# noegroup/bgflow

Measured on AMD Instinct MI355X. Metric: flow samples/s (fwd+log|detJ|) at batch 2^20, higher is better.
Workload: dtype f32 (split-f16 conditioner GEMMs: hi+lo f16 operand pairs, f32 accumulate)

## Files before the change

bgflow_amd/build.py:

```python
import glob
import os
import subprocess
import sys
from concurrent.futures import ThreadPoolExecutor

HERE = os.path.dirname(os.path.abspath(__file__))
CSRC = os.path.join(HERE, "csrc")
OBJ = os.path.join(CSRC, "build")
LIB = os.path.join(HERE, "libbgflow_amd.so")

HIPCC_FLAGS = [
    "--offload-arch=gfx950", "-O3", "-std=c++17", "-fPIC", "-fvisibility=hidden",
    "-ffp-contract=off", "-fhip-fp32-correctly-rounded-divide-sqrt", "-fno-fast-math",
    "-Wno-comment",
]
TU_FLAGS = {"bgk_fused2.hip": ["-fno-slp-vectorize"], "bgk_fused2_train.hip": ["-fno-slp-vectorize"],
            "bgk_fused2_bf16.hip": ["-fno-slp-vectorize"], "bgk_fused2_afftrain.hip": ["-fno-slp-vectorize"],
            "bgk_tail.hip": ["-fno-slp-vectorize"]}


INCLUDES_SOURCE = {"bgk_fused2_train.hip": ["bgk_fused2.hip"], "bgk_fused2_bf16.hip": ["bgk_fused2.hip"], "bgk_fused2_afftrain.hip": ["bgk_fused2.hip"]}


HEADER = os.path.join(HERE, "..", "include", "bgflow_amd.h")


def abi_symbols(header=HEADER):
    import re
    text = re.sub(r"/\*.*?\*/", "", open(header).read(), flags=re.S)
    return sorted(set(re.findall(r"^[A-Za-z_][\w \t\*]*?\b(bgk_\w+)\s*\(", text, flags=re.M)))


def _export_map():
    path = os.path.join(OBJ, "export.map")
    with open(path, "w") as f:
        f.write("{\n  global:\n" + "".join(f"    {n};\n" for n in abi_symbols()) + "  local:\n    *;\n};\n")
    return path


def sources():
    return sorted(glob.glob(os.path.join(CSRC, "*.hip")))


def _headers():
    return glob.glob(os.path.join(CSRC, "*.h")) + glob.glob(os.path.join(HERE, "..", "include", "*.h"))


def _obj(src, tag):
    return os.path.join(OBJ, os.path.basename(src) + tag + ".o")


def _stale():
    if not os.path.exists(LIB):
        return True
# ... 40 lines not shown
```

bgflow_amd/csrc/bgk_capi.hip:

```cpp
#include <stdarg.h>

#include "bgk_common.h"
#include "bgk_fused2.h"

extern int bgk_affine_variant;

static thread_local char g_err[512] = "";

void bgk_set_error(const char* fmt, ...) {
    va_list ap;
    va_start(ap, fmt);
    vsnprintf(g_err, sizeof(g_err), fmt, ap);
    va_end(ap);
}

extern "C" int bgk_abi_version(void) { return 1; }
extern "C" const char* bgk_last_error(void) { return g_err; }

extern "C" int bgk_set_option(int32_t option, int32_t value) {
    if (option == 1 && (value == 1 || value == 2)) {
        const int prev = bgk_h2_variant;
        bgk_h2_variant = value;
        return prev;
    }
    if (option == 2 && (value == 1 || value == 2)) {
        const int prev = bgk_affine_variant;
        bgk_affine_variant = value;
        return prev;
    }
    if (option == 3 && (value == 1 || value == 2)) {
        const int prev = bgk_rc_vjp_variant;
        bgk_rc_vjp_variant = value;
        return prev;
    }
    bgk_set_error("bgk_set_option: unknown option %d / value %d", option, value);
    return BGK_EINVAL;
}

namespace {
__global__ void detmath_probe_kernel(const float* x, int64_t n, int which, float* out) {
    int64_t i = (int64_t)blockIdx.x * blockDim.x + threadIdx.x;
    if (i >= n) return;
    float v = x[i], r;
    switch (which) {
        case 0: r = bgk_expf(v); break;
        case 1: r = bgk_logf(v); break;
        case 2: r = bgk_softplusf(v, 0.69384102162f); break;
        case 3: r = bgk_siluf(v); break;
        case 4: r = bgk_tanhf(v); break;
        default: r = v;
    }
    out[i] = r;
}
}

extern "C" int bgk_detmath_probe(const float* x, int64_t n, int32_t which, float* out, void* stream) {
    if (n <= 0) return 0;
    int grid = (int)((n + 255) / 256);
    hipLaunchKernelGGL(detmath_probe_kernel, dim3(grid), dim3(256), 0, (hipStream_t)stream, x, n, which, out);
    return bgk_launch_status("bgk_detmath_probe");
}
```

bgflow_amd/csrc/bgk_fused2.h:

```cpp
#ifndef BGK_FUSED2_H
#define BGK_FUSED2_H
#include <stdint.h>

#define BGK_MAX_COND 3
struct BgkCondSegs { const float* ptr[BGK_MAX_COND]; int64_t ld[BGK_MAX_COND]; int32_t w[BGK_MAX_COND]; int32_t n; };

int bgk_launch_rqs_dense_h2v2(const char* what, const float* cond, int64_t ldc, int32_t d_c, int32_t periodic,
                              const void* A0p, const void* A1p, const void* A2p, float c0, float c1, float c2, const float* cs_dev,
                              int32_t act, const float* y, int64_t ldy, int64_t B, int32_t d, uint64_t circ_mask, int32_t inverse,
                              double left, double right, double bottom, double top,
                              double min_bin_width, double min_bin_height, double min_derivative, int32_t identity_init,
                              float* out, int64_t ldo, float* dlogp, int32_t accumulate, int32_t* bin_idx, int32_t* oob_count,
                              void* stream, const BgkCondSegs* segs = nullptr, int32_t row_order = 1);

int bgk_launch_rqs_dense_h2v2_train(const char* what, float* z0, float* z1, float* params, int64_t ldp, const int32_t* src_col,
                                    const float* cond, int64_t ldc, int32_t d_c, int32_t periodic,
                                    const void* A0p, const void* A1p, const void* A2p, float c0, float c1, float c2, const float* cs_dev,
                                    int32_t act, const float* y, int64_t ldy, int64_t B, int32_t d, uint64_t circ_mask, int32_t inverse,
                                    double left, double right, double bottom, double top,
                                    double min_bin_width, double min_bin_height, double min_derivative, int32_t identity_init,
                                    float* out, int64_t ldo, float* dlogp, int32_t accumulate, int32_t* bin_idx, int32_t* oob_count,
                                    void* stream, const BgkCondSegs* segs = nullptr, int32_t row_order = 1);

int bgk_launch_rqs_bwd_recompute(const char* what, const float* z1, const void* A2p, float c2, const float* cs_dev, int32_t act,
                                 const float* y, int64_t ldy, int64_t B, int32_t d, uint64_t circ_mask, int32_t inverse,
                                 double left, double right, double bottom, double top,
                                 double min_bin_width, double min_bin_height, double min_derivative, int32_t identity_init,
                                 const float* g_out, int64_t ldgo, const float* g_dlogp, float* g_y, int64_t ldgy,
                                 float* g_params, int64_t ldgp, float* g_absmax, void* stream);

int bgk_launch_rqs_dense_h2v2_bf16(const char* what, const float* cond, int64_t ldc, int32_t d_c, int32_t periodic,
                                   const void* A0p, const void* A1p, const void* A2p, float c0, float c1, float c2, const float* cs_dev,
                                   int32_t act, const float* y, int64_t ldy, int64_t B, int32_t d, uint64_t circ_mask, int32_t inverse,
                                   double left, double right, double bottom, double top,
                                   double min_bin_width, double min_bin_height, double min_derivative, int32_t identity_init,
                                   float* out, int64_t ldo, float* dlogp, int32_t accumulate, int32_t* bin_idx, int32_t* oob_count,
                                   void* stream, const BgkCondSegs* segs = nullptr, int32_t row_order = 1);

int bgk_launch_affine_dense_v2(const float* cond, int64_t ldc, int32_t d_c, int32_t periodic,
                               const void* sA0, const void* sA1, const void* sA1b, const void* sA2, float sc0, float sc1, float sc1b, float sc2, int32_t s_act,
                               const void* tA0, const void* tA1, const void* tA1b, const void* tA2, float tc0, float tc1, float tc1b, float tc2, int32_t t_act,
                               const float* log_alpha, int32_t preserve_volume, int32_t is_circular, int32_t inverse,
                               const float* y, int64_t ldy, int64_t B, int32_t d,
                               float* out, int64_t ldo, float* dlogp, int32_t accumulate, void* stream, const BgkCondSegs* segs = nullptr);

struct BgkAffTrainSave { const float* s_cs; float* s_z0; float* s_z1; const float* t_cs; float* t_z0; float* t_z1; float* mu; float* s_raw; int64_t ldms;
                         int64_t ldz; };
int bgk_launch_affine_dense_v2_train(const BgkAffTrainSave* save, const float* cond, int64_t ldc, int32_t d_c, int32_t periodic,
                               const void* sA0, const void* sA1, const void* sA1b, const void* sA2, float sc0, float sc1, float sc1b, float sc2, int32_t s_act,
                               const void* tA0, const void* tA1, const void* tA1b, const void* tA2, float tc0, float tc1, float tc1b, float tc2, int32_t t_act,
                               const float* log_alpha, int32_t preserve_volume, int32_t is_circular, int32_t inverse,
                               const float* y, int64_t ldy, int64_t B, int32_t d,
                               float* out, int64_t ldo, float* dlogp, int32_t accumulate, void* stream, const BgkCondSegs* segs = nullptr);

extern int bgk_h2_variant;
extern int bgk_rc_vjp_variant;

#endif
```

bgflow_amd/csrc/bgk_fused2.hip:

```cpp
#include "bgk_common.h"
#include "bgk_fused2.h"

#ifndef BGK_V2_SAVE
#define BGK_V2_SAVE 0
#endif
#if BGK_V2_SAVE
#include "bgk_mfma_h2.h"
#include "bgk_rqs_vjp.h"
#define coupling_rqs_dense_h2v2_kernel coupling_rqs_dense_h2v2_train_kernel
#endif
#ifndef BGK_V2_BF16
#define BGK_V2_BF16 0
#endif
#if BGK_V2_BF16
#define coupling_rqs_dense_h2v2_kernel coupling_rqs_dense_h2v2_bf16_kernel
typedef short s16x8 __attribute__((ext_vector_type(8)));
#endif
#ifndef BGK_V2_AFFTRAIN
#define BGK_V2_AFFTRAIN 0
#endif
#if BGK_V2_AFFTRAIN
#define coupling_affine_dense_v2_kernel coupling_affine_dense_v2_train_kernel
#endif
constexpr int NPROD = BGK_V2_BF16 ? 1 : 3;

namespace {

typedef float f32x16 __attribute__((ext_vector_type(16)));
typedef _Float16 h16x8 __attribute__((ext_vector_type(8)));
typedef unsigned u32x4 __attribute__((ext_vector_type(4)));

constexpr int FW = 4;
constexpr int FTHREADS = FW * 64;
constexpr int KB = 8;
constexpr int PPD = 3 * KB + 1;
constexpr int DPC = 128 / PPD;
constexpr int SROW = 33;
constexpr int ST = BGK_V2_SAVE ? 33 : 32;
constexpr int KS = 8;
constexpr int GBLK = KS * 8 + 4;
#ifndef BGK_V2_KARG
#define BGK_V2_KARG 2
#endif
#ifndef BGK_V2_RD
#define BGK_V2_RD 4
#endif
#ifndef BGK_V2_TS
#define BGK_V2_TS 0
#endif
#if BGK_V2_TS
#define V2_TS(k) do { const unsigned long long t_ = __builtin_amdgcn_s_memtime(); if (lane == 0 && a.bin_idx) a.bin_idx[b0 * d + (k)] = (int)(unsigned)t_; } while (0)
#else
#define V2_TS(k) do { } while (0)
#endif
constexpr int RD = BGK_V2_RD;
constexpr int EH = 34;

struct CondSegs {
    const float* ptr[BGK_MAX_COND]; int64_t ld[BGK_MAX_COND]; int w[BGK_MAX_COND]; int off[BGK_MAX_COND]; uint32_t magic[BGK_MAX_COND];
    int n;
};

struct SetK { float gnum, low, high, dstep; float kc[7]; };

struct SpC {
    float left, right;
    SetK sa, sb;
    float beta, kout, min_d;
};

struct V2Args {
    CondSegs cs;
    int d_c; int periodic;
    const float* y; int64_t ldy; float* out; int64_t ldo; int d; uint32_t magic_d;
    int64_t B; float* dlogp; int accumulate; int32_t* bin_idx; int32_t* oob_count;
    const uint4* A0; const uint4* A1; const uint4* A2; int S0; int n_chunks; int last_tiles;
    float c0, c1, c2; const float* cs_dev;
    uint64_t circ_mask;
    SpC sc;
    int lds_per_wave;
    int nfs, ys, stage, y_dma, out_lin;
    int p_floats;
#if BGK_V2_SAVE
    float* z0; float* z1;
    float* params; int64_t ldp;
    const int32_t* src_col;
#endif
};
typedef const __attribute__((address_space(4))) V2Args* kargs_t;

struct BFrag { h16x8 hi[KS], lo[KS]; };
struct TFrag { u32x4 hi, lo; };

__device__ __forceinline__ int drow(int m, int r, int hh) { return 32 * m + (r & 3) + 8 * (r >> 2) + 4 * hh; }

template <int NT, int MS = 4, int RDX = RD>
struct Live {
    static constexpr int NTS = KS * NT;
    static constexpr int NEV = NPROD * NTS + NT;
    f32x16 (&out)[4];
    const BFrag& b;
    const uint4* W;
    unsigned voff;
    TFrag (&ring)[RDX];
    __amdgpu_buffer_rsrc_t rs;

    template <int BLK>
    __device__ __forceinline__ u32x4 blk() {
        return __builtin_amdgcn_raw_buffer_load_b128(rs, voff + ((BLK * 1024) & 4095), (BLK * 1024) & ~4095, 0);
    }
    template <int T>
    __device__ __forceinline__ void load() {
        if constexpr (T < NTS) {
            constexpr int s = T / NT, m = T % NT;
#if BGK_V2_BF16
// ... 559 lines not shown
    spline_slot_reg<INV, 2, 3 * EH>(g, a, k, h[2], s_p, s_y, c, DPC, hh, j, rows, run, oob_local, bins);
}

typedef const __attribute__((address_space(1))) void* gvp_t;
typedef __attribute__((address_space(3))) void* lvp_t;
__device__ __forceinline__ void dma_tile32(float* dst, const float* __restrict__ src, int n, int valid, int lane) {
    for (int c = 0; c < n; c += 256) {
        const int e = c + lane * 4;
        if (e + 3 < valid) __builtin_amdgcn_global_load_lds((gvp_t)(src + e), (lvp_t)(dst + c), 16, 0, 0);
    }
    if (valid & 3) {
        const int edge = valid & ~3;
        if (lane < (valid & 3)) __builtin_amdgcn_global_load_lds((gvp_t)(src + edge + lane), (lvp_t)(dst + edge), 4, 0, 0);
    }
}

__device__ __forceinline__ void v2_sincos2pi(float x, float* s, float* c) {
    const float f = __builtin_amdgcn_fractf(x);
    *s = __builtin_amdgcn_sinf(f);
    *c = __builtin_amdgcn_cosf(f);
}

struct StageTiles { int d_c, periodic, nfs, ys, stage, y_dma, d; uint32_t magic_d; int rows, lane; };

__device__ __forceinline__ void stage_issue(const StageTiles& t, const CondSegs& cs, int64_t b0, const float* y_t, float* s_p, float* s_y) {
    if (t.y_dma) dma_tile32(s_y, y_t, 32 * t.d, t.rows * t.d, t.lane);
    if (t.stage == 1) dma_tile32(s_p, cs.ptr[0] + b0 * cs.ld[0], 32 * t.d_c, t.rows * t.d_c, t.lane);
    else if (t.stage == 2) dma_tile32(s_p + 32 * t.nfs, cs.ptr[0] + b0 * cs.ld[0], 32 * t.d_c, t.rows * t.d_c, t.lane);
}

#ifndef BGK_V2_SB
#define BGK_V2_SB 8
#endif
template <class KA>
__device__ __forceinline__ void stage_finish(const StageTiles& t, const CondSegs& cs, int64_t b0, const float* y_t, int ldy32,
                                             float* s_p, float* s_y, float y_fill) {
    constexpr int SB = BGK_V2_SB;
    const int lane = t.lane, rows = t.rows, d = t.d, nfs = t.nfs, n_y = 32 * t.d;
    if (!t.y_dma) {
        for (int base = 0; base < n_y; base += 64 * SB) {
            float vy[SB];
#pragma unroll
            for (int u = 0; u < SB; ++u) {
                const int i = base + u * 64 + lane;
                const int r = (int)(__umul24((unsigned)i, t.magic_d) >> 20), c = i - (int)__umul24((unsigned)r, (unsigned)d);
                vy[u] = (i < n_y && r < rows) ? y_t[(int)__umul24((unsigned)r, (unsigned)ldy32) + c] : y_fill;
            }
#pragma unroll
            for (int u = 0; u < SB; ++u) {
                const int i = base + u * 64 + lane;
                const int r = (int)(__umul24((unsigned)i, t.magic_d) >> 20), c = i - (int)__umul24((unsigned)r, (unsigned)d);
                if (i < n_y) s_y[(int)__umul24((unsigned)r, (unsigned)t.ys) + c] = vy[u];
            }
        }
    }
    if (t.stage == 0) {
        typedef const __attribute__((address_space(4))) KA* ka_t;
        const ka_t kseg = (ka_t)__builtin_amdgcn_kernarg_segment_ptr();
        for (int sg = 0; sg < cs.n; ++sg) {
            const float* cond_t = kseg->cs.ptr[sg] + b0 * kseg->cs.ld[sg];
            const int ldc32 = (int)kseg->cs.ld[sg], w_c = kseg->cs.w[sg], n_c = 32 * w_c, col0 = kseg->cs.off[sg];
            const uint32_t magic_c = kseg->cs.magic[sg];
            for (int base = 0; base < n_c; base += 64 * SB) {
                float vc[SB];
#pragma unroll
                for (int u = 0; u < SB; ++u) {
                    const int i = base + u * 64 + lane;
                    const int r = (int)(__umul24((unsigned)i, magic_c) >> 20), c = i - (int)__umul24((unsigned)r, (unsigned)w_c);
                    vc[u] = (i < n_c && r < rows) ? cond_t[(int)__umul24((unsigned)r, (unsigned)ldc32) + c] : 0.0f;
                }
#pragma unroll
                for (int u = 0; u < SB; ++u) {
                    const int i = base + u * 64 + lane;
                    const int r = (int)(__umul24((unsigned)i, magic_c) >> 20), c = i - (int)__umul24((unsigned)r, (unsigned)w_c);
                    if (i < n_c) {
                        float* f = s_p + (int)__umul24((unsigned)r, (unsigned)nfs) + col0 + c;
                        if (t.periodic) {
                            float sv, cv;
                            v2_sincos2pi(vc[u], &sv, &cv);
                            f[0] = cv;
                            f[t.d_c] = sv;
                        } else {
                            f[0] = vc[u];
                        }
                    }
                }
            }
        }
    }
    asm volatile("s_waitcnt vmcnt(0)" ::: "memory");
    __builtin_amdgcn_fence(__ATOMIC_ACQ_REL, "wavefront");
    __builtin_amdgcn_wave_barrier();
    if (t.stage == 2) {
        const float* raw = s_p + 32 * nfs;
        const uint32_t magic_c = cs.magic[0];
        for (int i = lane; i < 32 * t.d_c; i += 64) {
            const int r = (int)(__umul24((unsigned)i, magic_c) >> 20), c = i - (int)__umul24((unsigned)r, (unsigned)t.d_c);
            float sv, cv;
            v2_sincos2pi(raw[i], &sv, &cv);
            float* f = s_p + (int)__umul24((unsigned)r, (unsigned)nfs) + c;
            f[0] = cv;
            f[t.d_c] = sv;
        }
    }
    if (t.stage != 1) {
        __builtin_amdgcn_fence(__ATOMIC_ACQ_REL, "wavefront");
        __builtin_amdgcn_wave_barrier();
    }
}

__device__ __forceinline__ void store_tile32(float* out_t, int ldo32, const float* s_y, int ys, int d, uint32_t magic_d, int rows, int lane, int lin) {
    const int n = rows * d;
    if (lin) {
        for (int i = lane * 4; i + 3 < n; i += 256) *reinterpret_cast<float4*>(out_t + i) = *reinterpret_cast<const float4*>(s_y + i);
        if (lane < (n & 3)) out_t[(n & ~3) + lane] = s_y[(n & ~3) + lane];
    } else {
        for (int i = lane; i < n; i += 64) {
            const int r = (int)(__umul24((unsigned)i, magic_d) >> 20), cc = i - (int)__umul24((unsigned)r, (unsigned)d);
            out_t[(int)__umul24((unsigned)r, (unsigned)ldo32) + cc] = s_y[(int)__umul24((unsigned)r, (unsigned)ys) + cc];
        }
    }
}

struct L0Frag { uint4 v[4][2]; };
__device__ __forceinline__ void l0_request(L0Frag& f, const uint4* A0, int s, int lane) {
// ... 10 lines not shown
#pragma unroll
    for (int e = 0; e < 8; ++e) v[e] = f[e];
    if (last) {
#pragma unroll
        for (int e = 0; e < 8; ++e) v[e] = rel0 + e == 0 ? 1.0f : (rel0 + e > 0 ? 0.0f : v[e]);
    }
#if BGK_V2_BF16
    s16x8 bb;
#pragma unroll
    for (int e = 0; e < 8; ++e) bb[e] = __builtin_bit_cast(short, (__bf16)v[e]);
#pragma unroll
    for (int m = 0; m < 4; ++m)
        h[m] = __builtin_amdgcn_mfma_f32_32x32x16_bf16(__builtin_bit_cast(s16x8, fr.v[m][0]), bb, h[m], 0, 0, 0);
#else
    h16x8 bhi, blo;
#pragma unroll
    for (int e = 0; e < 8; ++e) {
        const float c = v[e];
        const _Float16 hv = (_Float16)c;
        bhi[e] = hv;
        blo[e] = (_Float16)(c - (float)hv);
    }
#pragma unroll
    for (int m = 0; m < 4; ++m) h[m] = __builtin_amdgcn_mfma_f32_32x32x16_f16(__builtin_bit_cast(h16x8, fr.v[m][1]), bhi, h[m], 0, 0, 0);
#pragma unroll
    for (int m = 0; m < 4; ++m) h[m] = __builtin_amdgcn_mfma_f32_32x32x16_f16(__builtin_bit_cast(h16x8, fr.v[m][0]), blo, h[m], 0, 0, 0);
#pragma unroll
    for (int m = 0; m < 4; ++m) h[m] = __builtin_amdgcn_mfma_f32_32x32x16_f16(__builtin_bit_cast(h16x8, fr.v[m][0]), bhi, h[m], 0, 0, 0);
#endif
}

template <int ACT, int INV, bool SAVEP = true, bool REGP = false>
__global__ __launch_bounds__(FTHREADS, 2) void coupling_rqs_dense_h2v2_kernel(V2Args a) {
    static_assert(!REGP || (!BGK_V2_SAVE && !BGK_V2_BF16), "row order 2 belongs to the split-f16 inference instance");
    if (a.cs_dev) { a.c0 = a.cs_dev[1]; a.c1 = a.cs_dev[3]; a.c2 = a.cs_dev[5]; }
    asm volatile("s_setreg_imm32_b32 hwreg(HW_REG_MODE, 23, 1), 1");
    extern __shared__ __attribute__((aligned(16))) float smem[];
    const int wave = REGP ? __builtin_amdgcn_readfirstlane((int)(threadIdx.x >> 6)) : (int)(threadIdx.x >> 6);
    float* s_p = smem + (size_t)wave * a.lds_per_wave;
    float* s_y = s_p + (REGP ? a.p_floats : 128 * ST);
    const int d = a.d;
    const int64_t n_tiles = (a.B + 31) / 32;
    const int64_t tile = (int64_t)blockIdx.x * FW + wave;
    if (tile >= n_tiles) return;
    const SpK k{a.c2 * 1.44269504088896341f, a.c2 * a.sc.beta * 1.44269504088896341f, a.c2};
    const int n_in = a.periodic ? 2 * a.d_c : a.d_c;
    const int ldy32 = (int)a.ldy, ldo32 = (int)a.ldo;
    const int n_y = 32 * d;

  {
    const int lane = (int)threadIdx.x & 63, j = lane & 31, hh = lane >> 5;
    const unsigned voff = (unsigned)lane * 16u;
    const int64_t b0 = tile * 32;
    const int rows = (int)((a.B - b0) < 32 ? (a.B - b0) : 32);
    const float* y_t = a.y + b0 * a.ldy;
    float* out_t = a.out + b0 * a.ldo;
    V2_TS(0);

    const int nfs = a.nfs, ys = a.ys;
    const StageTiles stg{a.d_c, a.periodic, nfs, ys, a.stage, a.y_dma, d, a.magic_d, rows, lane};
    stage_issue(stg, a.cs, b0, y_t, s_p, s_y);
    f32x16 h[4], acc[4];
    TFrag ring[RD];
    BFrag bf;
    L0Frag fa, fb;
    l0_request(fa, a.A0, 0, lane);
    Live<4> g1{acc, bf, a.A1, voff, ring};
    g1.start();
    V2_TS(12);
    stage_finish<V2Args>(stg, a.cs, b0, y_t, ldy32, s_p, s_y, 0.5f);
    V2_TS(1);

#pragma unroll
    for (int m = 0; m < 4; ++m)
#pragma unroll
        for (int r = 0; r < 16; ++r) h[m][r] = 0.0f;
    {
        const float* frow = s_p + j * nfs + 8 * hh;
        const int rel0 = 16 * (a.S0 - 1) + 8 * hh - n_in;
        for (int s = 0; s < a.S0; s += 2) {
            if (s + 1 < a.S0) l0_request(fb, a.A0, s + 1, lane);
            l0_step(h, fa, frow + 16 * s, s + 1 == a.S0, rel0);
            if (s + 1 < a.S0) {
                if (s + 2 < a.S0) l0_request(fa, a.A0, s + 2, lane);
                l0_step(h, fb, frow + 16 * (s + 1), s + 2 == a.S0, rel0);
            }
        }
    }

    V2_TS(2);
    {
        Live<4>& g = g1;
#if BGK_V2_SAVE
#pragma unroll
        for (int m = 0; m < 4; ++m)
#pragma unroll
            for (int r = 0; r < 16; ++r) h[m][r] *= a.c0;
        h2_store_rows128(h, a.z0, s_p, b0, rows, lane);
        const float c0_act = 1.0f;
#else
        const float c0_act = a.c0;
#endif
        NoLive none;
// ... 38 lines not shown
        int bins[3] = {0, 0, 0};
        const int nd = (d - c * DPC) < DPC ? (d - c * DPC) : DPC;
        if constexpr (REGP) {
            if (c + 2 < a.n_chunks || (c + 2 == a.n_chunks && a.last_tiles > 2)) {
                chunk_piped_reg<INV, 4>(a, k, s_p, s_y, c, hh, j, rows, run, oob_local, bins, h, bf, ring, voff);
            } else if (c + 2 == a.n_chunks) {
                chunk_piped_reg<INV, 2>(a, k, s_p, s_y, c, hh, j, rows, run, oob_local, bins, h, bf, ring, voff);
            } else {
                NoLive none;
                slab_to_lds(h, s_p, hh, j);
                spline_slot_reg<INV, 0, 1>(none, a, k, h[0], s_p, s_y, c, nd, hh, j, rows, run, oob_local, bins);
                if (nd > 2) spline_slot_reg<INV, 1, 1>(none, a, k, h[2], s_p, s_y, c, nd, hh, j, rows, run, oob_local, bins);
                if (nd > 4) spline_slot_reg<INV, 2, 1>(none, a, k, h[2], s_p, s_y, c, nd, hh, j, rows, run, oob_local, bins);
            }
        } else
        if (c + 2 < a.n_chunks || (c + 2 == a.n_chunks && a.last_tiles > 2)) {
            chunk_piped<INV, 4, SAVEP>(a, k, s_p, s_y, c, hh, j, rows, run, oob_local, bins, h, bf, ring, voff, b0);
        } else if (c + 2 == a.n_chunks) {
            chunk_piped<INV, 2, SAVEP>(a, k, s_p, s_y, c, hh, j, rows, run, oob_local, bins, h, bf, ring, voff, b0);
        } else {
            NoLive none;
            chunk_to_lds(h, s_p, hh, j);
#if BGK_V2_SAVE
            if constexpr (SAVEP) save_chunk_params(a, s_p, c, lane, b0, rows);
#endif
            spline_slot<INV, 0, 1>(none, a, k, s_p, s_y, c, nd, hh, j, rows, run, oob_local, bins);
            if (nd > 2) spline_slot<INV, 1, 1>(none, a, k, s_p, s_y, c, nd, hh, j, rows, run, oob_local, bins);
            if (nd > 4) spline_slot<INV, 2, 1>(none, a, k, s_p, s_y, c, nd, hh, j, rows, run, oob_local, bins);
        }
#if BGK_V2_TS
        V2_TS(5 + c);
#else
        if (a.bin_idx) {
#pragma unroll
            for (int it = 0; it < 3; ++it) {
                const int q = 2 * it + hh;
                if (q < nd && j < rows) a.bin_idx[(b0 + j) * d + c * DPC + q] = bins[it];
            }
        }
#endif
        __builtin_amdgcn_fence(__ATOMIC_ACQ_REL, "wavefront");
        __builtin_amdgcn_wave_barrier();
    }
    int lane_e = lane;
    if constexpr (REGP) {
        int zero = 0;
        asm volatile("" : "+v"(zero));
        lane_e = (int)__builtin_amdgcn_mbcnt_hi(~0u, __builtin_amdgcn_mbcnt_lo(~0u, (unsigned)zero));
    }
    if ((lane_e >> 5) == 0 && (lane_e & 31) < rows) {
        if (a.accumulate) a.dlogp[b0 + (lane_e & 31)] += run; else a.dlogp[b0 + (lane_e & 31)] = run;
    }
    store_tile32(out_t, ldo32, s_y, ys, d, a.magic_d, rows, lane_e, a.out_lin);
    if (a.oob_count && __builtin_amdgcn_ballot_w64(oob_local != 0)) {
        for (int off = 32; off > 0; off >>= 1) oob_local += __shfl_xor(oob_local, off);
        if (lane_e == 0) atomicAdd(a.oob_count, oob_local);
    }
    V2_TS(5 + a.n_chunks);
  }
}

struct TilePlan { int nfs, ys, stage, y_dma, out_lin; };
TilePlan plan_tiles(const CondSegs& cs, int d_c, int periodic, const float* y, int64_t ldy, const float* out, int64_t ldo, int d, int tile_floats) {
    const int n_in = periodic ? 2 * d_c : d_c;
    const auto dma_ok = [](const float* p, int64_t ld, int w) { return ld == w && ((uintptr_t)p & 15) == 0 && (w & 7) != 0; };
    TilePlan t;
    t.y_dma = dma_ok(y, ldy, d) ? 1 : 0;
    t.ys = t.y_dma ? d : (d | 1);
    t.out_lin = (t.y_dma && ldo == d && ((uintptr_t)out & 15) == 0) ? 1 : 0;
    const bool c_dma = cs.n == 1 && dma_ok(cs.ptr[0], cs.ld[0], d_c);
    t.stage = (c_dma && !periodic) ? 1 : ((c_dma && periodic && 32 * ((n_in | 1) + d_c) <= tile_floats) ? 2 : 0);
    t.nfs = t.stage == 1 ? d_c : (n_in | 1);
    return t;
}

SetK make_set(double low, double high, double min_bin, int K) {
    SetK s;
    const double span = high - low, scale = 1.0 - min_bin * K;
    s.gnum = (float)((double)(float)span * (double)(float)scale);
    s.low = (float)low; s.high = (float)high;
    s.dstep = (float)((double)(float)span * (double)(float)min_bin);
    for (int k = 0; k < 7; ++k) s.kc[k] = (float)((double)(float)low + (double)(float)span * (double)(float)min_bin * (k + 1));
    return s;
}

uint32_t magic_div(int d) { return (uint32_t)(((1u << 20) + (uint32_t)d - 1) / (uint32_t)d); }

bool make_cond_segs(CondSegs& cs, const float* cond, int64_t ldc, int d_c, const BgkCondSegs* segs) {
    for (int i = 0; i < BGK_MAX_COND; ++i) { cs.ptr[i] = nullptr; cs.ld[i] = 0; cs.w[i] = 0; cs.off[i] = 0; cs.magic[i] = 0; }
    if (!segs || segs->n <= 1) {
        const float* p = segs && segs->n == 1 ? segs->ptr[0] : cond;
        const int64_t ld = segs && segs->n == 1 ? segs->ld[0] : ldc;
        if (!p || d_c <= 0 || ld >= (1 << 24)) return false;
        cs.n = 1; cs.ptr[0] = p; cs.ld[0] = ld; cs.w[0] = d_c; cs.magic[0] = magic_div(d_c);
        return true;
    }
    if (segs->n > BGK_MAX_COND) return false;
    int off = 0;
    for (int i = 0; i < segs->n; ++i) {
        if (!segs->ptr[i] || segs->w[i] <= 0 || segs->ld[i] < segs->w[i] || segs->ld[i] >= (1 << 24)) return false;
        cs.ptr[i] = segs->ptr[i]; cs.ld[i] = segs->ld[i]; cs.w[i] = segs->w[i]; cs.off[i] = off; cs.magic[i] = magic_div(segs->w[i]);
        off += segs->w[i];
    }
    cs.n = segs->n;
    return off == d_c;
}


#if !BGK_V2_SAVE && !BGK_V2_BF16
struct AffV2Net { const uint4* A0; const uint4* A1; const uint4* A1b; const uint4* A2; float c0, c1, c1b, c2;
#if BGK_V2_AFFTRAIN
                  const float* cs;
                  float* z0; float* z1;
#endif
};
struct AffV2Args {
    CondSegs cs; int d_c; int periodic; int S0;
    AffV2Net shift, scale; int has_shift, has_scale;
    const float* log_alpha; int preserve_volume, is_circular, inverse;
    const float* y; int64_t ldy; int64_t B; int d;
    float* out; int64_t ldo; float* dlogp; int accumulate;
    uint32_t magic_d;
    int lds_tile, lds_per_wave;
    int nfs, ys, stage, y_dma, out_lin;
#if BGK_V2_AFFTRAIN
    float* mu_out; float* s_out; int64_t ldms;
    int slab;
    int zt;
#endif
};

#if BGK_V2_AFFTRAIN
template <int NT>
__device__ __forceinline__ void aff_store_tiles(const f32x16 (&t)[4], float* dst, int pitch, float* slab, int64_t b0, int rows, int lane) {
    const int j = lane & 31, hh = lane >> 5;
    const __amdgpu_buffer_rsrc_t rs = __builtin_amdgcn_make_buffer_rsrc((void*)(dst + b0 * pitch), 0, rows * pitch * 4, 0x00020000);
#pragma unroll
    for (int m = 0; m < NT; ++m)
#pragma unroll
        for (int half = 0; half < 2; ++half) {
            if ((j >> 4) == half) {
#pragma unroll
// ... 450 lines not shown
    const float gl = (a.g_dlogp + b0)[jr];
    float gmax = 0.0f;
    const RcTile tl{__builtin_amdgcn_make_buffer_rsrc((void*)(a.y + b0 * a.ldy), 0, (int)(rows * a.ldy * 4), 0x00020000),
                    __builtin_amdgcn_make_buffer_rsrc((void*)(a.g_out + b0 * a.ldgo), 0, (int)(rows * a.ldgo * 4), 0x00020000),
                    __builtin_amdgcn_make_buffer_rsrc((void*)(a.g_y + b0 * a.ldgy), 0, (int)(rows * a.ldgy * 4), 0x00020000),
                    __builtin_amdgcn_make_buffer_rsrc((void*)(a.g_params + b0 * a.ldgp), 0, (int)(rows * a.ldgp * 4), 0x00020000),
                    jr * (int)a.ldy * 4, jr * (int)a.ldgo * 4, j * (int)a.ldgy * 4};
    RcIn in = rc_request(tl, 0, 0, a.d < DPC ? a.d : DPC, hh);
    for (int c = 0; c + 1 < a.n_chunks; ++c) {
        if (c + 2 < a.n_chunks || a.last_tiles > 2) rc_chunk<4, 3, FAST>(a, tl, s_p, c, DPC, lane, rows, gl, gmax, in, h, bf, ring, voff, ts);
        else rc_chunk<2, 3, FAST>(a, tl, s_p, c, DPC, lane, rows, gl, gmax, in, h, bf, ring, voff, ts);
    }
    {
        const int c = a.n_chunks - 1, nd = a.d - c * DPC;
        if (nd > 4) rc_chunk<0, 3, FAST>(a, tl, s_p, c, nd, lane, rows, gl, gmax, in, h, bf, ring, voff, ts);
        else if (nd > 2) rc_chunk<0, 2, FAST>(a, tl, s_p, c, nd, lane, rows, gl, gmax, in, h, bf, ring, voff, ts);
        else rc_chunk<0, 1, FAST>(a, tl, s_p, c, nd, lane, rows, gl, gmax, in, h, bf, ring, voff, ts);
    }
    bgk_publish_absmax(a.g_absmax, gmax);
#if BGK_RC_TS
    asm volatile("s_waitcnt vmcnt(0)" ::: "memory");
    unsigned q4;
    RC_Q(q4);
    if (lane == 0) {
        unsigned* o = reinterpret_cast<unsigned*>(a.g_y + b0 * a.ldgy);
        o[0] = q1 - q0; o[1] = q2 - q1; o[2] = q3 - q2; o[3] = ts.lds; o[4] = ts.vjp; o[5] = ts.gemm; o[6] = ts.st; o[7] = q4 - q0;
    }
#endif
}
#endif

}

#if !BGK_V2_SAVE && !BGK_V2_BF16 && !BGK_V2_AFFTRAIN
int bgk_h2_variant = 2;
#endif

#if BGK_V2_SAVE
int bgk_rc_vjp_variant = 2;
int bgk_launch_rqs_bwd_recompute(const char* what, const float* z1, const void* A2p, float c2, const float* cs_dev, int32_t act,
                                 const float* y, int64_t ldy, int64_t B, int32_t d, uint64_t circ_mask, int32_t inverse,
                                 double left, double right, double bottom, double top,
                                 double min_bin_width, double min_bin_height, double min_derivative, int32_t identity_init,
                                 const float* g_out, int64_t ldgo, const float* g_dlogp, float* g_y, int64_t ldgy,
                                 float* g_params, int64_t ldgp, float* g_absmax, void* stream) {
    RcArgs a;
    a.z1 = z1; a.A2 = reinterpret_cast<const uint4*>(A2p); a.c2 = c2; a.cs_dev = cs_dev;
    a.n_chunks = (d + DPC - 1) / DPC;
    a.last_tiles = ((d - (a.n_chunks - 1) * DPC) * PPD + 31) / 32;
    a.y = y; a.ldy = ldy; a.B = B; a.d = d; a.nc_mask = ~circ_mask & (d >= 64 ? ~0ull : ((1ull << d) - 1ull)); a.inverse = inverse;
    BGK_CHECK_ARG(ldy < (1 << 24) && ldgo < (1 << 24) && ldgy < (1 << 24) && ldgp < (1 << 24), "%s: row stride too large", what);
    a.g_out = g_out; a.ldgo = ldgo; a.g_dlogp = g_dlogp; a.g_y = g_y; a.ldgy = ldgy; a.g_params = g_params; a.ldgp = ldgp;
    a.g_absmax = g_absmax;
    a.cfg = bgk_make_rqs_cfg(left, right, bottom, top, min_bin_width, min_bin_height, min_derivative, identity_init, KB);
    a.lds_per_wave = ((128 * ST + 3) / 4) * 4;
    static_assert(128 * ST >= 32 * 128, "the chunk buffer holds the z1 tile");
    const size_t shmem = sizeof(float) * (size_t)FW * a.lds_per_wave;
    const int64_t n_wg = ((B + 31) / 32 + FW - 1) / FW;
    BGK_CHECK_ARG(n_wg < (int64_t)0x7fffffff, "%s: batch too large for one launch", what);
    hipStream_t st = (hipStream_t)stream;
#define BGK_LAUNCH(A, F) do { (void)hipFuncSetAttribute(reinterpret_cast<const void*>(coupling_rqs_bwd_recompute_kernel<A, F>), hipFuncAttributeMaxDynamicSharedMemorySize, 160 * 1024); \
                              hipLaunchKernelGGL((coupling_rqs_bwd_recompute_kernel<A, F>), dim3((int)n_wg), dim3(FTHREADS), shmem, st, a); } while (0)
#define BGK_LAUNCH_F(A) do { if (bgk_rc_vjp_variant == 1) BGK_LAUNCH(A, false); else BGK_LAUNCH(A, true); } while (0)
    if (act == 1) BGK_LAUNCH_F(1); else if (act == 2) BGK_LAUNCH_F(2); else BGK_LAUNCH_F(3);
#undef BGK_LAUNCH_F
#undef BGK_LAUNCH
    return bgk_launch_status(what);
}
#endif

#if !BGK_V2_AFFTRAIN
#if BGK_V2_SAVE
int bgk_launch_rqs_dense_h2v2_train(const char* what, float* z0, float* z1, float* params, int64_t ldp, const int32_t* src_col,
                                    const float* cond, int64_t ldc, int32_t d_c, int32_t periodic,
#elif BGK_V2_BF16
int bgk_launch_rqs_dense_h2v2_bf16(const char* what, const float* cond, int64_t ldc, int32_t d_c, int32_t periodic,
#else
int bgk_launch_rqs_dense_h2v2(const char* what, const float* cond, int64_t ldc, int32_t d_c, int32_t periodic,
#endif
                              const void* A0p, const void* A1p, const void* A2p, float c0, float c1, float c2, const float* cs_dev,
                              int32_t act, const float* y, int64_t ldy, int64_t B, int32_t d, uint64_t circ_mask, int32_t inverse,
                              double left, double right, double bottom, double top,
                              double min_bin_width, double min_bin_height, double min_derivative, int32_t identity_init,
                              float* out, int64_t ldo, float* dlogp, int32_t accumulate, int32_t* bin_idx, int32_t* oob_count,
                              void* stream, const BgkCondSegs* segs, int32_t row_order) {
    V2Args a;
#if BGK_V2_SAVE || BGK_V2_BF16
    BGK_CHECK_ARG(row_order == 1, "%s: output-layer row order %d (this instance takes order 1)", what, row_order);
    constexpr bool regp = false;
#else
    BGK_CHECK_ARG(row_order == 1 || row_order == 2, "%s: output-layer row order %d (1 | 2)", what, row_order);
    const bool regp = row_order == 2;
#endif
    const int n_in = periodic ? 2 * d_c : d_c;
    BGK_CHECK_ARG(make_cond_segs(a.cs, cond, ldc, d_c, segs), "%s: bad conditioning segments", what);
    a.d_c = d_c; a.periodic = periodic;
    a.y = y; a.ldy = ldy; a.out = out; a.ldo = ldo; a.d = d; a.magic_d = magic_div(d);
    a.B = B; a.dlogp = dlogp; a.accumulate = accumulate; a.bin_idx = bin_idx; a.oob_count = oob_count;
    a.A0 = reinterpret_cast<const uint4*>(A0p); a.A1 = reinterpret_cast<const uint4*>(A1p); a.A2 = reinterpret_cast<const uint4*>(A2p);
    a.S0 = (n_in + 1 + 15) / 16;
    a.n_chunks = (d + DPC - 1) / DPC;
    a.last_tiles = ((d - (a.n_chunks - 1) * DPC) * PPD + 31) / 32;
    a.c0 = c0; a.c1 = c1; a.c2 = c2; a.cs_dev = cs_dev;
    a.circ_mask = circ_mask;
    a.sc.left = (float)left; a.sc.right = (float)right;
    const SetK sw = make_set(left, right, min_bin_width, KB), sh = make_set(bottom, top, min_bin_height, KB);
    a.sc.sa = inverse ? sw : sh;
    a.sc.sb = inverse ? sh : sw;
    const double beta = identity_init ? (0.6931471805599453 / (1.0 - min_derivative)) : 1.0;
    a.sc.beta = (float)beta; a.sc.kout = (float)(0.6931471805599453 / (double)(float)beta); a.sc.min_d = (float)min_derivative;
    const TilePlan tp = plan_tiles(a.cs, d_c, periodic, y, ldy, out, ldo, d, 128 * ST);
    a.nfs = tp.nfs; a.ys = tp.ys; a.stage = tp.stage; a.y_dma = tp.y_dma; a.out_lin = tp.out_lin;
    BGK_CHECK_ARG(32 * a.nfs + 16 <= 128 * ST, "%s: %d conditioner input features do not fit the LDS tile", what, n_in);
    a.p_floats = 128 * ST;
    if (regp) {
        const int feat = 32 * a.nfs + (a.stage == 2 ? 32 * d_c : 0) + 16;
        a.p_floats = ((feat > SLAB ? feat : SLAB) + 3) / 4 * 4;
    }
    a.lds_per_wave = ((a.p_floats + 32 * a.ys + 32 + 3) / 4) * 4;
#if BGK_V2_SAVE
    a.z0 = z0; a.z1 = z1; a.params = params; a.ldp = ldp; a.src_col = src_col;
#endif
    const size_t shmem = sizeof(float) * (size_t)FW * a.lds_per_wave;
    const int64_t n_wg = ((B + 31) / 32 + FW - 1) / FW;
    BGK_CHECK_ARG(n_wg < (int64_t)0x7fffffff, "%s: batch too large for one launch", what);
    BGK_CHECK_ARG((int64_t)32 * (d > d_c ? d : d_c) < (1 << 16), "%s: tile index range", what);
    BGK_CHECK_ARG(ldy < (1 << 24) && ldo < (1 << 24), "%s: row stride too large", what);
    const int grid = (int)n_wg;
    hipStream_t st = (hipStream_t)stream;
#if BGK_V2_SAVE
#define BGK_LAUNCH(A, I) do { if (params) hipLaunchKernelGGL((coupling_rqs_dense_h2v2_kernel<A, I, true>), dim3(grid), dim3(FTHREADS), shmem, st, a); \
                              else hipLaunchKernelGGL((coupling_rqs_dense_h2v2_kernel<A, I, false>), dim3(grid), dim3(FTHREADS), shmem, st, a); } while (0)
#elif BGK_V2_BF16
#define BGK_LAUNCH(A, I) hipLaunchKernelGGL((coupling_rqs_dense_h2v2_kernel<A, I>), dim3(grid), dim3(FTHREADS), shmem, st, a)
#else
#define BGK_LAUNCH(A, I) do { if (regp) hipLaunchKernelGGL((coupling_rqs_dense_h2v2_kernel<A, I, true, true>), dim3(grid), dim3(FTHREADS), shmem, st, a); \
                              else hipLaunchKernelGGL((coupling_rqs_dense_h2v2_kernel<A, I>), dim3(grid), dim3(FTHREADS), shmem, st, a); } while (0)
#endif
    if (act == 1) { if (inverse) BGK_LAUNCH(1, 1); else BGK_LAUNCH(1, 0); }
    else if (act == 2) { if (inverse) BGK_LAUNCH(2, 1); else BGK_LAUNCH(2, 0); }
    else { if (inverse) BGK_LAUNCH(3, 1); else BGK_LAUNCH(3, 0); }
#undef BGK_LAUNCH
    return bgk_launch_status(what);
}
#endif

#if !BGK_V2_SAVE && !BGK_V2_BF16
#if BGK_V2_AFFTRAIN
int bgk_launch_affine_dense_v2_train(const BgkAffTrainSave* save,
                               const float* cond, int64_t ldc, int32_t d_c, int32_t periodic,
#else
int bgk_launch_affine_dense_v2(const float* cond, int64_t ldc, int32_t d_c, int32_t periodic,
#endif
                               const void* sA0, const void* sA1, const void* sA1b, const void* sA2, float sc0, float sc1, float sc1b, float sc2, int32_t s_act,
                               const void* tA0, const void* tA1, const void* tA1b, const void* tA2, float tc0, float tc1, float tc1b, float tc2, int32_t t_act,
                               const float* log_alpha, int32_t preserve_volume, int32_t is_circular, int32_t inverse,
                               const float* y, int64_t ldy, int64_t B, int32_t d,
                               float* out, int64_t ldo, float* dlogp, int32_t accumulate, void* stream, const BgkCondSegs* segs) {
#if BGK_V2_AFFTRAIN
    const char* what = "bgk_coupling_affine_dense_h2_train";
#else
    const char* what = "bgk_coupling_affine_dense_h2";
#endif
    AffV2Args a;
    const int n_in = periodic ? 2 * d_c : d_c;
    BGK_CHECK_ARG(make_cond_segs(a.cs, cond, ldc, d_c, segs), "%s: bad conditioning segments", what);
    a.d_c = d_c; a.periodic = periodic; a.S0 = (n_in + 1 + 15) / 16;
#if BGK_V2_AFFTRAIN
    a.shift = AffV2Net{(const uint4*)sA0, (const uint4*)sA1, (const uint4*)sA1b, (const uint4*)sA2, sc0, sc1, sc1b, sc2, save->s_cs, save->s_z0, save->s_z1};
    a.scale = AffV2Net{(const uint4*)tA0, (const uint4*)tA1, (const uint4*)tA1b, (const uint4*)tA2, tc0, tc1, tc1b, tc2, save->t_cs, save->t_z0, save->t_z1};
    a.mu_out = save->mu; a.s_out = save->s_raw; a.ldms = save->ldms; a.zt = save->ldz == 64 ? 2 : 4;
#else
    a.shift = AffV2Net{(const uint4*)sA0, (const uint4*)sA1, (const uint4*)sA1b, (const uint4*)sA2, sc0, sc1, sc1b, sc2};
    a.scale = AffV2Net{(const uint4*)tA0, (const uint4*)tA1, (const uint4*)tA1b, (const uint4*)tA2, tc0, tc1, tc1b, tc2};
#endif
    a.has_shift = sA0 != nullptr; a.has_scale = tA0 != nullptr;
    const bool deep = a.has_shift ? sA1b != nullptr : tA1b != nullptr;
#if BGK_V2_AFFTRAIN
    if (deep) return BGK_EUNSUPPORTED;
    BGK_CHECK_ARG((!a.has_shift || (save->s_z0 && save->s_z1 && save->mu)) && (!a.has_scale || (save->t_z0 && save->t_z1 && save->s_raw)),
// ... 48 lines not shown
```

Measured before the change: 133.7 million.

## Make row-order-2 RQS coupling kernel persistent with grid-stride tile loop

Moves the row-order-2 (register-parameter) RQS coupling kernel into its own translation unit and turns it into a persistent kernel. The grid is capped at two workgroups per CU, and each wave loops over tiles with a stride. Kernel arguments are reloaded from the kernarg segment on every iteration, and asm barriers are used to keep register pressure in check. This aims to cut workgroup launch and tail overhead, but it serialises tiles inside each wave, which can reduce latency hiding and makes the code more complex.

```diff
diff --git a/bgflow_amd/build.py b/bgflow_amd/build.py
--- a/bgflow_amd/build.py
+++ b/bgflow_amd/build.py
@@ -16,10 +16,11 @@
 ]
 TU_FLAGS = {"bgk_fused2.hip": ["-fno-slp-vectorize"], "bgk_fused2_train.hip": ["-fno-slp-vectorize"],
             "bgk_fused2_bf16.hip": ["-fno-slp-vectorize"], "bgk_fused2_afftrain.hip": ["-fno-slp-vectorize"],
+            "bgk_fused2_regp.hip": ["-fno-slp-vectorize", "-mllvm", "-disable-machine-licm"],
             "bgk_tail.hip": ["-fno-slp-vectorize"]}
 
 
-INCLUDES_SOURCE = {"bgk_fused2_train.hip": ["bgk_fused2.hip"], "bgk_fused2_bf16.hip": ["bgk_fused2.hip"], "bgk_fused2_afftrain.hip": ["bgk_fused2.hip"]}
+INCLUDES_SOURCE = {"bgk_fused2_regp.hip": ["bgk_fused2.hip"], "bgk_fused2_train.hip": ["bgk_fused2.hip"], "bgk_fused2_bf16.hip": ["bgk_fused2.hip"], "bgk_fused2_afftrain.hip": ["bgk_fused2.hip"]}
 
 
 HEADER = os.path.join(HERE, "..", "include", "bgflow_amd.h")
diff --git a/bgflow_amd/csrc/bgk_capi.hip b/bgflow_amd/csrc/bgk_capi.hip
--- a/bgflow_amd/csrc/bgk_capi.hip
+++ b/bgflow_amd/csrc/bgk_capi.hip
@@ -33,6 +33,11 @@
         bgk_rc_vjp_variant = value;
         return prev;
     }
+    if (option == 4 && value >= 0) {
+        const int prev = bgk_persist_wg_cap;
+        bgk_persist_wg_cap = value;
+        return prev;
+    }
     bgk_set_error("bgk_set_option: unknown option %d / value %d", option, value);
     return BGK_EINVAL;
 }
diff --git a/bgflow_amd/csrc/bgk_fused2.h b/bgflow_amd/csrc/bgk_fused2.h
--- a/bgflow_amd/csrc/bgk_fused2.h
+++ b/bgflow_amd/csrc/bgk_fused2.h
@@ -12,6 +12,14 @@
                               double min_bin_width, double min_bin_height, double min_derivative, int32_t identity_init,
                               float* out, int64_t ldo, float* dlogp, int32_t accumulate, int32_t* bin_idx, int32_t* oob_count,
                               void* stream, const BgkCondSegs* segs = nullptr, int32_t row_order = 1);
+
+int bgk_launch_rqs_dense_h2v2_regp(const char* what, const float* cond, int64_t ldc, int32_t d_c, int32_t periodic,
+                                   const void* A0p, const void* A1p, const void* A2p, float c0, float c1, float c2, const float* cs_dev,
+                                   int32_t act, const float* y, int64_t ldy, int64_t B, int32_t d, uint64_t circ_mask, int32_t inverse,
+                                   double left, double right, double bottom, double top,
+                                   double min_bin_width, double min_bin_height, double min_derivative, int32_t identity_init,
+                                   float* out, int64_t ldo, float* dlogp, int32_t accumulate, int32_t* bin_idx, int32_t* oob_count,
+                                   void* stream, const BgkCondSegs* segs = nullptr, int32_t row_order = 2);
 
 int bgk_launch_rqs_dense_h2v2_train(const char* what, float* z0, float* z1, float* params, int64_t ldp, const int32_t* src_col,
                                     const float* cond, int64_t ldc, int32_t d_c, int32_t periodic,
@@ -54,6 +62,7 @@
                                float* out, int64_t ldo, float* dlogp, int32_t accumulate, void* stream, const BgkCondSegs* segs = nullptr);
 
 extern int bgk_h2_variant;
+extern int bgk_persist_wg_cap;
 extern int bgk_rc_vjp_variant;
 
 #endif
diff --git a/bgflow_amd/csrc/bgk_fused2.hip b/bgflow_amd/csrc/bgk_fused2.hip
--- a/bgflow_amd/csrc/bgk_fused2.hip
+++ b/bgflow_amd/csrc/bgk_fused2.hip
@@ -15,6 +15,9 @@
 #if BGK_V2_BF16
 #define coupling_rqs_dense_h2v2_kernel coupling_rqs_dense_h2v2_bf16_kernel
 typedef short s16x8 __attribute__((ext_vector_type(8)));
+#endif
+#ifndef BGK_V2_REGP
+#define BGK_V2_REGP 0
 #endif
 #ifndef BGK_V2_AFFTRAIN
 #define BGK_V2_AFFTRAIN 0
@@ -81,6 +84,7 @@
     int lds_per_wave;
     int nfs, ys, stage, y_dma, out_lin;
     int p_floats;
+    int tile_stride;
 #if BGK_V2_SAVE
     float* z0; float* z1;
     float* params; int64_t ldp;
@@ -706,9 +710,10 @@
 #ifndef BGK_V2_SB
 #define BGK_V2_SB 8
 #endif
-template <class KA>
+struct NoStamp { __device__ __forceinline__ void operator()(int) const {} };
+template <class KA, class TS = NoStamp>
 __device__ __forceinline__ void stage_finish(const StageTiles& t, const CondSegs& cs, int64_t b0, const float* y_t, int ldy32,
-                                             float* s_p, float* s_y, float y_fill) {
+                                             float* s_p, float* s_y, float y_fill, TS ts = TS()) {
     constexpr int SB = BGK_V2_SB;
     const int lane = t.lane, rows = t.rows, d = t.d, nfs = t.nfs, n_y = 32 * t.d;
     if (!t.y_dma) {
@@ -762,9 +767,11 @@
             }
         }
     }
+    ts(0);
     asm volatile("s_waitcnt vmcnt(0)" ::: "memory");
     __builtin_amdgcn_fence(__ATOMIC_ACQ_REL, "wavefront");
     __builtin_amdgcn_wave_barrier();
+    ts(1);
     if (t.stage == 2) {
         const float* raw = s_p + 32 * nfs;
         const uint32_t magic_c = cs.magic[0];
@@ -841,29 +848,42 @@
 
 template <int ACT, int INV, bool SAVEP = true, bool REGP = false>
 __global__ __launch_bounds__(FTHREADS, 2) void coupling_rqs_dense_h2v2_kernel(V2Args a) {
-    static_assert(!REGP || (!BGK_V2_SAVE && !BGK_V2_BF16), "row order 2 belongs to the split-f16 inference instance");
-    if (a.cs_dev) { a.c0 = a.cs_dev[1]; a.c1 = a.cs_dev[3]; a.c2 = a.cs_dev[5]; }
+    static_assert(REGP == (BGK_V2_REGP != 0), "row order 2 belongs to the split-f16 inference instance of bgk_fused2_regp.hip");
+    constexpr bool PERSIST = REGP;
+    if constexpr (!PERSIST) {
+        if (a.cs_dev) { a.c0 = a.cs_dev[1]; a.c1 = a.cs_dev[3]; a.c2 = a.cs_dev[5]; }
+    }
     asm volatile("s_setreg_imm32_b32 hwreg(HW_REG_MODE, 23, 1), 1");
     extern __shared__ __attribute__((aligned(16))) float smem[];
     const int wave = REGP ? __builtin_amdgcn_readfirstlane((int)(threadIdx.x >> 6)) : (int)(threadIdx.x >> 6);
-    float* s_p = smem + (size_t)wave * a.lds_per_wave;
-    float* s_y = s_p + (REGP ? a.p_floats : 128 * ST);
+    float* const s_p = smem + (size_t)wave * a.lds_per_wave;
+    int64_t tile = (int64_t)blockIdx.x * FW + wave;
+    if (tile >= (a.B + 31) / 32) return;
+    bool more = false;
+
+  do {
+    if constexpr (PERSIST) {
+        kargs_t ka = (kargs_t)__builtin_amdgcn_kernarg_segment_ptr();
+        asm volatile("" : "+s"(ka));
+        a = *(const V2Args*)ka;
+        if (a.cs_dev) { a.c0 = a.cs_dev[1]; a.c1 = a.cs_dev[3]; a.c2 = a.cs_dev[5]; }
+    }
+    float* const s_y = s_p + (REGP ? a.p_floats : 128 * ST);
     const int d = a.d;
-    const int64_t n_tiles = (a.B + 31) / 32;
-    const int64_t tile = (int64_t)blockIdx.x * FW + wave;
-    if (tile >= n_tiles) return;
     const SpK k{a.c2 * 1.44269504088896341f, a.c2 * a.sc.beta * 1.44269504088896341f, a.c2};
     const int n_in = a.periodic ? 2 * a.d_c : a.d_c;
-    const int ldy32 = (int)a.ldy, ldo32 = (int)a.ldo;
-    const int n_y = 32 * d;
-
-  {
-    const int lane = (int)threadIdx.x & 63, j = lane & 31, hh = lane >> 5;
+    const int ldy32 = (int)a.ldy;
+    int lane = (int)threadIdx.x & 63;
+    if constexpr (PERSIST) {
+        int zero = 0;
+        asm volatile("" : "+v"(zero));
+        lane = (int)__builtin_amdgcn_mbcnt_hi(~0u, __builtin_amdgcn_mbcnt_lo(~0u, (unsigned)zero));
+    }
+    const int j = lane & 31, hh = lane >> 5;
     const unsigned voff = (unsigned)lane * 16u;
     const int64_t b0 = tile * 32;
     const int rows = (int)((a.B - b0) < 32 ? (a.B - b0) : 32);
     const float* y_t = a.y + b0 * a.ldy;
-    float* out_t = a.out + b0 * a.ldo;
     V2_TS(0);
 
     const int nfs = a.nfs, ys = a.ys;
@@ -873,11 +893,19 @@
     TFrag ring[RD];
     BFrag bf;
     L0Frag fa, fb;
+    if constexpr (PERSIST) {
+#pragma unroll
+        for (int m = 0; m < 4; ++m) { asm volatile("" : "=v"(fb.v[m][0])); asm volatile("" : "=v"(fb.v[m][1])); }
+    }
     l0_request(fa, a.A0, 0, lane);
     Live<4> g1{acc, bf, a.A1, voff, ring};
     g1.start();
     V2_TS(12);
+#if BGK_V2_TS
+    stage_finish<V2Args>(stg, a.cs, b0, y_t, ldy32, s_p, s_y, 0.5f, [&](int i) { V2_TS(10 + i); });
+#else
     stage_finish<V2Args>(stg, a.cs, b0, y_t, ldy32, s_p, s_y, 0.5f);
+#endif
     V2_TS(1);
 
 #pragma unroll
@@ -982,10 +1010,20 @@
         V2_TS(5 + c);
 #else
         if (a.bin_idx) {
-#pragma unroll
-            for (int it = 0; it < 3; ++it) {
-                const int q = 2 * it + hh;
-                if (q < nd && j < rows) a.bin_idx[(b0 + j) * d + c * DPC + q] = bins[it];
+            if constexpr (PERSIST) {
+                int jo = j, ho = hh;
+                asm volatile("" : "+v"(jo), "+v"(ho));
+                int32_t* bt = a.bin_idx + b0 * d;
+                const unsigned off = (unsigned)(jo * d + c * DPC + ho);
+#pragma unroll
+                for (int it = 0; it < 3; ++it)
+                    if (2 * it + ho < nd && jo < rows) bt[off + 2u * it] = bins[it];
+            } else {
+#pragma unroll
+                for (int it = 0; it < 3; ++it) {
+                    const int q = 2 * it + hh;
+                    if (q < nd && j < rows) a.bin_idx[(b0 + j) * d + c * DPC + q] = bins[it];
+                }
             }
         }
 #endif
@@ -998,16 +1036,36 @@
         asm volatile("" : "+v"(zero));
         lane_e = (int)__builtin_amdgcn_mbcnt_hi(~0u, __builtin_amdgcn_mbcnt_lo(~0u, (unsigned)zero));
     }
-    if ((lane_e >> 5) == 0 && (lane_e & 31) < rows) {
-        if (a.accumulate) a.dlogp[b0 + (lane_e & 31)] += run; else a.dlogp[b0 + (lane_e & 31)] = run;
-    }
-    store_tile32(out_t, ldo32, s_y, ys, d, a.magic_d, rows, lane_e, a.out_lin);
-    if (a.oob_count && __builtin_amdgcn_ballot_w64(oob_local != 0)) {
-        for (int off = 32; off > 0; off >>= 1) oob_local += __shfl_xor(oob_local, off);
-        if (lane_e == 0) atomicAdd(a.oob_count, oob_local);
+    V2Args a_tail;
+    if constexpr (PERSIST) {
+        kargs_t kb = (kargs_t)__builtin_amdgcn_kernarg_segment_ptr();
+        asm volatile("" : "+s"(kb));
+        a_tail = *(const V2Args*)kb;
+    }
+    const V2Args& t = PERSIST ? a_tail : a;
+    const int64_t b0t = tile * 32;
+    const int rows_t = (int)((t.B - b0t) < 32 ? (t.B - b0t) : 32);
+    if ((lane_e >> 5) == 0 && (lane_e & 31) < rows_t) {
+        if (t.accumulate) t.dlogp[b0t + (lane_e & 31)] += run; else t.dlogp[b0t + (lane_e & 31)] = run;
+    }
+    store_tile32(t.out + b0t * t.ldo, (int)t.ldo, s_p + (REGP ? t.p_floats : 128 * ST), t.ys, t.d, t.magic_d, rows_t, lane_e, t.out_lin);
+    if (t.oob_count && __builtin_amdgcn_ballot_w64(oob_local != 0)) {
+        if constexpr (PERSIST) {
+            for (int off = 32; off > 0; off >>= 1) oob_local += __builtin_amdgcn_ds_bpermute((lane_e ^ off) << 2, oob_local);
+        } else {
+            for (int off = 32; off > 0; off >>= 1) oob_local += __shfl_xor(oob_local, off);
+        }
+        if (lane_e == 0) atomicAdd(t.oob_count, oob_local);
     }
     V2_TS(5 + a.n_chunks);
-  }
+    if constexpr (PERSIST) {
+        asm volatile("s_waitcnt lgkmcnt(0)" ::: "memory");
+        __builtin_amdgcn_fence(__ATOMIC_ACQ_REL, "wavefront");
+        __builtin_amdgcn_wave_barrier();
+        tile += t.tile_stride;
+        more = tile < (t.B + 31) / 32;
+    }
+  } while (PERSIST && more);
 }
 
 struct TilePlan { int nfs, ys, stage, y_dma, out_lin; };
@@ -1057,7 +1115,7 @@
 }
 
 
-#if !BGK_V2_SAVE && !BGK_V2_BF16
+#if !BGK_V2_SAVE && !BGK_V2_BF16 && !BGK_V2_REGP
 struct AffV2Net { const uint4* A0; const uint4* A1; const uint4* A1b; const uint4* A2; float c0, c1, c1b, c2;
 #if BGK_V2_AFFTRAIN
                   const float* cs;
@@ -1574,8 +1632,27 @@
 
 }
 
-#if !BGK_V2_SAVE && !BGK_V2_BF16 && !BGK_V2_AFFTRAIN
+#if !BGK_V2_SAVE && !BGK_V2_BF16 && !BGK_V2_AFFTRAIN && !BGK_V2_REGP
 int bgk_h2_variant = 2;
+#endif
+#if BGK_V2_REGP
+int bgk_persist_wg_cap = 0;
+
+namespace {
+int resident_workgroups() {
+    static int cached[64];
+    int dev = 0;
+    if (hipGetDevice(&dev) != hipSuccess || dev < 0 || dev >= 64) return 0;
+    int v = __atomic_load_n(&cached[dev], __ATOMIC_RELAXED);
+    if (v == 0) {
+        int cus = 0;
+        if (hipDeviceGetAttribute(&cus, hipDeviceAttributeMultiprocessorCount, dev) != hipSuccess || cus <= 0) return 0;
+        v = 2 * cus;
+        __atomic_store_n(&cached[dev], v, __ATOMIC_RELAXED);
+    }
+    return v;
+}
+}
 #endif
 
 #if BGK_V2_SAVE
@@ -1617,6 +1694,8 @@
                                     const float* cond, int64_t ldc, int32_t d_c, int32_t periodic,
 #elif BGK_V2_BF16
 int bgk_launch_rqs_dense_h2v2_bf16(const char* what, const float* cond, int64_t ldc, int32_t d_c, int32_t periodic,
+#elif BGK_V2_REGP
+int bgk_launch_rqs_dense_h2v2_regp(const char* what, const float* cond, int64_t ldc, int32_t d_c, int32_t periodic,
 #else
 int bgk_launch_rqs_dense_h2v2(const char* what, const float* cond, int64_t ldc, int32_t d_c, int32_t periodic,
 #endif
@@ -1626,14 +1705,21 @@
                               double min_bin_width, double min_bin_height, double min_derivative, int32_t identity_init,
                               float* out, int64_t ldo, float* dlogp, int32_t accumulate, int32_t* bin_idx, int32_t* oob_count,
                               void* stream, const BgkCondSegs* segs, int32_t row_order) {
-    V2Args a;
 #if BGK_V2_SAVE || BGK_V2_BF16
     BGK_CHECK_ARG(row_order == 1, "%s: output-layer row order %d (this instance takes order 1)", what, row_order);
     constexpr bool regp = false;
+#elif BGK_V2_REGP
+    BGK_CHECK_ARG(row_order == 2, "%s: output-layer row order %d (this instance takes order 2)", what, row_order);
+    constexpr bool regp = true;
 #else
     BGK_CHECK_ARG(row_order == 1 || row_order == 2, "%s: output-layer row order %d (1 | 2)", what, row_order);
-    const bool regp = row_order == 2;
-#endif
+    if (row_order == 2)
+        return bgk_launch_rqs_dense_h2v2_regp(what, cond, ldc, d_c, periodic, A0p, A1p, A2p, c0, c1, c2, cs_dev, act, y, ldy, B, d, circ_mask, inverse,
+                                              left, right, bottom, top, min_bin_width, min_bin_height, min_derivative, identity_init,
+                                              out, ldo, dlogp, accumulate, bin_idx, oob_count, stream, segs, row_order);
+    constexpr bool regp = false;
+#endif
+    V2Args a;
     const int n_in = periodic ? 2 * d_c : d_c;
     BGK_CHECK_ARG(make_cond_segs(a.cs, cond, ldc, d_c, segs), "%s: bad conditioning segments", what);
     a.d_c = d_c; a.periodic = periodic;
@@ -1664,8 +1750,17 @@
     a.z0 = z0; a.z1 = z1; a.params = params; a.ldp = ldp; a.src_col = src_col;
 #endif
     const size_t shmem = sizeof(float) * (size_t)FW * a.lds_per_wave;
-    const int64_t n_wg = ((B + 31) / 32 + FW - 1) / FW;
+    int64_t n_wg = ((B + 31) / 32 + FW - 1) / FW;
     BGK_CHECK_ARG(n_wg < (int64_t)0x7fffffff, "%s: batch too large for one launch", what);
+#if BGK_V2_REGP
+    if (regp) {
+        int64_t slots = resident_workgroups();
+        BGK_CHECK_ARG(slots > 0, "%s: cannot read the device's CU count", what);
+        if (bgk_persist_wg_cap > 0 && bgk_persist_wg_cap < slots) slots = bgk_persist_wg_cap;
+        if (n_wg > slots) n_wg = slots;
+    }
+#endif
+    a.tile_stride = regp ? (int)n_wg * FW : 0;
     BGK_CHECK_ARG((int64_t)32 * (d > d_c ? d : d_c) < (1 << 16), "%s: tile index range", what);
     BGK_CHECK_ARG(ldy < (1 << 24) && ldo < (1 << 24), "%s: row stride too large", what);
     const int grid = (int)n_wg;
@@ -1675,9 +1770,10 @@
                               else hipLaunchKernelGGL((coupling_rqs_dense_h2v2_kernel<A, I, false>), dim3(grid), dim3(FTHREADS), shmem, st, a); } while (0)
 #elif BGK_V2_BF16
 #define BGK_LAUNCH(A, I) hipLaunchKernelGGL((coupling_rqs_dense_h2v2_kernel<A, I>), dim3(grid), dim3(FTHREADS), shmem, st, a)
-#else
-#define BGK_LAUNCH(A, I) do { if (regp) hipLaunchKernelGGL((coupling_rqs_dense_h2v2_kernel<A, I, true, true>), dim3(grid), dim3(FTHREADS), shmem, st, a); \
-                              else hipLaunchKernelGGL((coupling_rqs_dense_h2v2_kernel<A, I>), dim3(grid), dim3(FTHREADS), shmem, st, a); } while (0)
+#elif BGK_V2_REGP
+#define BGK_LAUNCH(A, I) hipLaunchKernelGGL((coupling_rqs_dense_h2v2_kernel<A, I, true, true>), dim3(grid), dim3(FTHREADS), shmem, st, a)
+#else
+#define BGK_LAUNCH(A, I) hipLaunchKernelGGL((coupling_rqs_dense_h2v2_kernel<A, I>), dim3(grid), dim3(FTHREADS), shmem, st, a)
 #endif
     if (act == 1) { if (inverse) BGK_LAUNCH(1, 1); else BGK_LAUNCH(1, 0); }
     else if (act == 2) { if (inverse) BGK_LAUNCH(2, 1); else BGK_LAUNCH(2, 0); }
@@ -1687,7 +1783,7 @@
 }
 #endif
 
-#if !BGK_V2_SAVE && !BGK_V2_BF16
+#if !BGK_V2_SAVE && !BGK_V2_BF16 && !BGK_V2_REGP
 #if BGK_V2_AFFTRAIN
 int bgk_launch_affine_dense_v2_train(const BgkAffTrainSave* save,
                                const float* cond, int64_t ldc, int32_t d_c, int32_t periodic,
diff --git a/bgflow_amd/csrc/bgk_fused2_regp.hip b/bgflow_amd/csrc/bgk_fused2_regp.hip
--- /dev/null
+++ b/bgflow_amd/csrc/bgk_fused2_regp.hip
@@ -0,0 +1,2 @@
+#define BGK_V2_REGP 1
+#include "bgk_fused2.hip"
```

New measurement: 123.5 million. 7.6% lower.
